# haotiansun14/rl-rep

Hardware: NVIDIA B200
Metric: agent updates/sec (higher is better)
Workload: dtype tf32

## Files before the change

### rlrep_b200/csrc/gemm_chain.cu

```cuda
#include <algorithm>
#include <cmath>
#include <cstdlib>
#include <cstring>

#include "common.cuh"
#include "gemm_chain.cuh"
#include "ptx.cuh"

namespace rlrep {

namespace {

constexpr int kThreads = 320;
constexpr int kEpiWarps = 8;
constexpr int kStages = 6;
constexpr int kCW = 16;
constexpr int kTwPitch = kCW + 4;
constexpr int kMaxBn = 128;
constexpr int kBM = 128, kBK = 32;
constexpr int kABytes = kBM * kBK * 4;
constexpr int kStageBytes = kABytes + kMaxBn * kBK * 4;
constexpr int kTbufFloats = kEpiWarps * 32 * kTwPitch;
constexpr int kSub = 4, kCtrStride = 32;
constexpr int kDbgItems = 16, kDbgEvents = 10;
constexpr int kSmemBytes = kStages * kStageBytes + 1024 + 256 + kTbufFloats * 4;
static_assert(kSmemBytes <= 227 * 1024, "chain kernel shared memory");

__device__ __forceinline__ void red_release_add(unsigned* p, unsigned v) {
  asm volatile("red.release.gpu.global.add.u32 [%0], %1;" ::"l"(p), "r"(v) : "memory");
}
__device__ __forceinline__ unsigned atom_add_acq_rel(unsigned* p, unsigned v) {
  unsigned old;
  asm volatile("atom.acq_rel.gpu.global.add.u32 %0, [%1], %2;" : "=r"(old) : "l"(p), "r"(v) : "memory");
  return old;
}
__device__ __forceinline__ void fence_proxy_async_global() { asm volatile("fence.proxy.async.global;" ::: "memory"); }
__device__ __forceinline__ void fence_tensormap_acquire(const CUtensorMap* m) {
  asm volatile("fence.proxy.tensormap::generic.acquire.gpu [%0], 128;" ::"l"(reinterpret_cast<uint64_t>(m)) : "memory");
}
__device__ __forceinline__ unsigned ld_relaxed(const unsigned* p) {
  unsigned v;
  asm volatile("ld.relaxed.gpu.global.u32 %0, [%1];" : "=r"(v) : "l"(p) : "memory");
  return v;
}
__device__ __forceinline__ void wait_counter(const unsigned* done, int dep, int dep_tiles) {
  const unsigned* p = done + (size_t)dep * kSub * kCtrStride;
  unsigned target[kSub];
#pragma unroll
  for (int sub = 0; sub < kSub; ++sub) target[sub] = (unsigned)((dep_tiles - sub + kSub - 1) / kSub);
  long long t0 = 0;
  while (true) {
    unsigned v[kSub];
#pragma unroll
    for (int sub = 0; sub < kSub; ++sub) v[sub] = ld_relaxed(p + sub * kCtrStride);
    bool ok = true;
#pragma unroll
    for (int sub = 0; sub < kSub; ++sub) ok = ok && v[sub] >= target[sub];
    if (ok) return;
    __nanosleep(20);
    if (t0 == 0) t0 = clock64();
    if (clock64() - t0 > 4000000000LL) {
      printf("rlrep: chain dependency wait timed out (block %d, gemm %d, tiles %d, counters %u %u %u %u)\n", blockIdx.x, dep,
             dep_tiles, v[0], v[1], v[2], v[3]);
      __trap();
    }
  }
}
__device__ __forceinline__ void fence_acquire_gpu() { asm volatile("fence.acq_rel.gpu;" ::: "memory"); }

__device__ __forceinline__ void epilogue_bar() { asm volatile("bar.sync 1, 256;" ::: "memory"); }

__device__ __forceinline__ float elu_fast(float x) {
  const float n = fminf(x, 0.f);
  float p = 1.f / 5040.f;
  p = fmaf(p, n, 1.f / 720.f);
  p = fmaf(p, n, 1.f / 120.f);
  p = fmaf(p, n, 1.f / 24.f);
  p = fmaf(p, n, 1.f / 6.f);
  p = fmaf(p, n, 0.5f);
  p = fmaf(p, n, 1.f);
  p *= n;
  const float e = __expf(n) - 1.f;
  const float r = n < -0.34657359f ? e : p;
  return x > 0.f ? x : r;
}

__device__ __forceinline__ bool aligned16(const void* p) { return (reinterpret_cast<uintptr_t>(p) & 15) == 0; }

__device__ __forceinline__ float chain_epilogue_scalar(const Epilogue& e, float acc, int m, int n, const float* cptr) {
  float v = acc * e.scale;
  if (e.r1_u) v = fmaf(__ldcg(e.r1_u + m), __ldcg(e.r1_v + n), v);
  if (e.bias) v += __ldg(e.bias + n);
  if (e.pre_out) e.pre_out[(size_t)m * e.ld_pre + n] = v;
  v = apply_act(v, e.act);
  if (e.dact != DACT_NONE) v *= apply_dact(__ldcg(e.aux + (size_t)m * e.ld_aux + n), e.dact);
  if (e.accumulate) v += __ldcg(cptr);
  return v;
}

struct ChunkOperands {
  float4 bias, r1v;
  float4 aux[4];
  float r1u[4];
};
__device__ __forceinline__ void chunk_prefetch(ChunkOperands& o, const Epilogue& epi, int M, int m_base, int gn0, int lane) {
  const int piece = lane & 3, rsub = lane >> 2;
  const int on = gn0 + 4 * piece;
  o.bias = make_float4(0.f, 0.f, 0.f, 0.f);
  o.r1v = make_float4(0.f, 0.f, 0.f, 0.f);
  if (epi.bias) o.bias = __ldg(reinterpret_cast<const float4*>(epi.bias + on));
  if (epi.r1_u) o.r1v = __ldcg(reinterpret_cast<const float4*>(epi.r1_v + on));
#pragma unroll
  for (int r4 = 0; r4 < 4; ++r4) {
    const int om = m_base + r4 * 8 + rsub;
    o.aux[r4] = make_float4(0.f, 0.f, 0.f, 0.f);
    o.r1u[r4] = 0.f;
    if (om < M) {
      if (epi.dact != DACT_NONE) o.aux[r4] = __ldcg(reinterpret_cast<const float4*>(epi.aux + (size_t)om * epi.ld_aux + on));
      if (epi.r1_u) o.r1u[r4] = __ldcg(epi.r1_u + om);
    }
  }
}

template <int ACT, int DACT>
__device__ __forceinline__ void chain_store_rows(const Epilogue& epi, const ChunkOperands& o, const float* tw,
                                                 float* __restrict__ C, int ldc, int M, int m_base, int gn0, int lane) {
  const int piece = lane & 3, rsub = lane >> 2;
  const int on = gn0 + 4 * piece;
#pragma unroll
  for (int r4 = 0; r4 < 4; ++r4) {
    const int r = r4 * 8 + rsub;
    const int om = m_base + r;
    if (om < M) {
      const float4 a4 = *reinterpret_cast<const float4*>(tw + r * kTwPitch + 4 * piece);
      float v[4] = {a4.x * epi.scale, a4.y * epi.scale, a4.z * epi.scale, a4.w * epi.scale};
      if (epi.r1_u) {
        const float u = o.r1u[r4];
        v[0] = fmaf(u, o.r1v.x, v[0]); v[1] = fmaf(u, o.r1v.y, v[1]); v[2] = fmaf(u, o.r1v.z, v[2]); v[3] = fmaf(u, o.r1v.w, v[3]);
      }
      v[0] += o.bias.x; v[1] += o.bias.y; v[2] += o.bias.z; v[3] += o.bias.w;
      if (epi.pre_out)
        *reinterpret_cast<float4*>(epi.pre_out + (size_t)om * epi.ld_pre + on) = make_float4(v[0], v[1], v[2], v[3]);
      if constexpr (ACT != ACT_NONE) {
#pragma unroll
        for (int e = 0; e < 4; ++e) v[e] = ACT == ACT_ELU ? elu_fast(v[e]) : apply_act(v[e], ACT < 0 ? epi.act : ACT);
      }
      if constexpr (DACT != DACT_NONE) {
        const int dact = DACT < 0 ? epi.dact : DACT;
        if (dact != DACT_NONE) {
          const float4 x = o.aux[r4];
          v[0] *= apply_dact(x.x, dact); v[1] *= apply_dact(x.y, dact); v[2] *= apply_dact(x.z, dact); v[3] *= apply_dact(x.w, dact);
        }
      }
      float4* cp = reinterpret_cast<float4*>(C + (size_t)om * ldc + on);
      if (epi.accumulate) {
        const float4 c0 = __ldcg(cp);
        v[0] += c0.x; v[1] += c0.y; v[2] += c0.z; v[3] += c0.w;
      }
      *cp = make_float4(v[0], v[1], v[2], v[3]);
    }
  }
}

__global__ void __launch_bounds__(kThreads, 1)
gemm_chain_kernel(const ChainGemmDesc* __restrict__ gemms, const ChainTask* __restrict__ tasks,
                  const int* __restrict__ task_begin, unsigned* __restrict__ done, unsigned* __restrict__ exit_ctr,
                  int n_gemms, unsigned long long* __restrict__ dbg) {
  auto stamp = [&](int item, int ev) {
    if (dbg != nullptr && item < kDbgItems) {
      unsigned long long t;
      asm volatile("mov.u64 %0, %%globaltimer;" : "=l"(t)::"memory");
      dbg[((size_t)blockIdx.x * kDbgItems + item) * kDbgEvents + ev] = t;
    }
  };
  if (threadIdx.x == 0) stamp(kDbgItems - 1, 2);
  extern __shared__ uint8_t smem_raw[];
  uint8_t* smem = reinterpret_cast<uint8_t*>((reinterpret_cast<uintptr_t>(smem_raw) + 1023) & ~uintptr_t(1023));
  uint64_t* full_bar = reinterpret_cast<uint64_t*>(smem + kStages * kStageBytes);
  uint64_t* empty_bar = full_bar + 8;
  uint64_t* acc_full = empty_bar + 8;
  uint64_t* acc_empty = acc_full + 2;
  uint32_t* tmem_slot = reinterpret_cast<uint32_t*>(acc_empty + 2);
  volatile unsigned* arrival = reinterpret_cast<volatile unsigned*>(tmem_slot + 1);
  float* tbuf = reinterpret_cast<float*>(smem + kStages * kStageBytes + 256);

  const int warp = threadIdx.x >> 5, lane = threadIdx.x & 31;
  const int t_begin = task_begin[blockIdx.x], t_end = task_begin[blockIdx.x + 1];

  if (threadIdx.x == 0) {
    for (int s = 0; s < kStages; ++s) {
      ptx::mbar_init(&full_bar[s], 1);
      ptx::mbar_init(&empty_bar[s], 1);
    }
    for (int a = 0; a < 2; ++a) {
      ptx::mbar_init(&acc_full[a], 1);
      ptx::mbar_init(&acc_empty[a], kEpiWarps);
    }
    ptx::fence_mbar_init();
  }
  if (warp == 1) {
    ptx::tmem_alloc(tmem_slot, 2 * kMaxBn);
    ptx::tmem_relinquish();
  }
  ptx::tc_fence_before_sync();
  __syncthreads();
  ptx::tc_fence_after_sync();
  const uint32_t tmem_base = *tmem_slot;
  ptx::pdl_wait();

  if (warp == 0) {
    if (lane == 0) {
      int it = 0, last_gemm = -1;
      for (int t = t_begin; t < t_end; ++t) {
        const ChainTask tk = tasks[t];
        const ChainGemmDesc* g = gemms + tk.gemm;
        const int n_deps = g->n_deps;
        const int bn = g->bn, a_mn = g->a_mn, b_mn = g->b_mn;
        const int m0 = (tk.tile % g->tiles_m) * kBM, n0 = (tk.tile / g->tiles_m) * bn;
        const int kb0 = tk.split * g->kb_per_split, kb1 = min(g->nkb, kb0 + g->kb_per_split);
        int dep_id[kChainMaxDeps], dep_tiles[kChainMaxDeps];
#pragma unroll
        for (int d = 0; d < kChainMaxDeps; ++d) {
          dep_id[d] = d < n_deps ? g->dep[d] : 0;
          dep_tiles[d] = d < n_deps ? (int)g->dep_target[d] : 0;
        }
        if (tk.gemm != last_gemm) {
          fence_tensormap_acquire(&g->tmA);
          fence_tensormap_acquire(&g->tmB);
          last_gemm = tk.gemm;
        }
        stamp(t - t_begin, 0);
        if (dbg != nullptr && t - t_begin < kDbgItems)
          dbg[((size_t)blockIdx.x * kDbgItems + (t - t_begin)) * kDbgEvents + 8] =
              (unsigned long long)tk.gemm | ((unsigned long long)tk.tile << 16) | ((unsigned long long)tk.split << 40);
#pragma unroll
        for (int d = 0; d < kChainMaxDeps; ++d)
          if (d < n_deps) wait_counter(done, dep_id[d], dep_tiles[d]);
        if (n_deps > 0) {
          fence_acquire_gpu();
          fence_proxy_async_global();
        }
        stamp(t - t_begin, 1);
        const uint32_t tx = kABytes + bn * kBK * 4;
        for (int kb = kb0; kb < kb1; ++kb, ++it) {
          const int s = it % kStages;
          ptx::mbar_wait(&empty_bar[s], ((it / kStages) & 1) ^ 1);
          ptx::mbar_arrive_expect_tx(&full_bar[s], tx);
          uint8_t* a_dst = smem + s * kStageBytes;
          uint8_t* b_dst = a_dst + kABytes;
          const int k0 = kb * kBK;
          if (!a_mn) ptx::tma_load_2d(a_dst, &g->tmA, &full_bar[s], k0, m0);
          else ptx::tma_load_3d(a_dst, &g->tmA, &full_bar[s], 0, k0, m0 / 32);
          if (!b_mn) ptx::tma_load_2d(b_dst, &g->tmB, &full_bar[s], k0, n0);
          else ptx::tma_load_3d(b_dst, &g->tmB, &full_bar[s], 0, k0, n0 / 32);
        }
        stamp(t - t_begin, 2);
      }
    }
  } else if (warp == 1) {
    if (ptx::elect_one()) {
      int it = 0, tc = 0;
      for (int t = t_begin; t < t_end; ++t, ++tc) {
        const ChainTask tk = tasks[t];
        const ChainGemmDesc* g = gemms + tk.gemm;
        const int bn = g->bn, a_mn = g->a_mn, b_mn = g->b_mn;
        const int kb0 = tk.split * g->kb_per_split, kb1 = min(g->nkb, kb0 + g->kb_per_split);
        const uint32_t idesc = ptx::make_idesc_tf32(kBM, bn, a_mn != 0, b_mn != 0);
        const int acc = tc & 1;
        ptx::mbar_wait(&acc_empty[acc], ((tc >> 1) & 1) ^ 1);
        ptx::tc_fence_after_sync();
        const uint32_t d_tmem = tmem_base + acc * kMaxBn;
        for (int kb = kb0; kb < kb1; ++kb, ++it) {
          const int s = it % kStages;
          ptx::mbar_wait(&full_bar[s], (it / kStages) & 1);
          if (kb == kb0) stamp(t - t_begin, 3);
          ptx::tc_fence_after_sync();
          const uint32_t a_addr = ptx::smem_u32(smem + s * kStageBytes);
          const uint32_t b_addr = a_addr + kABytes;
#pragma unroll
          for (int k = 0; k < kBK / 8; ++k) {
            const uint64_t adesc = a_mn ? ptx::make_smem_desc(a_addr + k * 1024, 4096, 512, 1)
                                        : ptx::make_smem_desc(a_addr + k * 32, 16, 1024, 2);
            const uint64_t bdesc = b_mn ? ptx::make_smem_desc(b_addr + k * 1024, 4096, 512, 1)
                                        : ptx::make_smem_desc(b_addr + k * 32, 16, 1024, 2);
            ptx::mma_tf32_ss(d_tmem, adesc, bdesc, idesc, (kb > kb0 || k > 0) ? 1u : 0u);
          }
          ptx::mma_commit(&empty_bar[s]);
        }
        ptx::mma_commit(&acc_full[acc]);
        stamp(t - t_begin, 4);
      }
    }
  } else {
    const int q = warp & 3, half = (warp - 2) >> 2;
    float* tw = tbuf + (warp - 2) * (32 * kTwPitch);
    int tc = 0;
    for (int t = t_begin; t < t_end; ++t, ++tc) {
      const ChainTask tk = tasks[t];
      const ChainGemmDesc* g = gemms + tk.gemm;
      const Epilogue epi = g->epi;
      const int bn = g->bn, M = g->M, N = g->N, ldc = g->ldc, split_k = g->split_k;
      float* __restrict__ C = g->C;
      float* __restrict__ ws = g->ws;
      unsigned* __restrict__ tile_ctr = g->tile_ctr;
      const int m0 = (tk.tile % g->tiles_m) * kBM, n0 = (tk.tile / g->tiles_m) * bn;
      const int chunks = bn / kCW;
      const int acc = tc & 1;
      const uint32_t t_acc = tmem_base + (static_cast<uint32_t>(32 * q) << 16) + acc * kMaxBn;
      const int row = 32 * q + lane;
      ptx::mbar_wait(&acc_full[acc], (tc >> 1) & 1);
      if (threadIdx.x == 64) stamp(t - t_begin, 5);
      ptx::tc_fence_after_sync();

      bool final = true;
      const size_t part_floats = (size_t)kBM * bn;
      float* ws_tile = split_k > 1 ? ws + (size_t)tk.tile * split_k * part_floats : nullptr;
      const bool dist = split_k > 1 && g->dist != 0;
      int c_first = half, c_step = 2;
      if (split_k > 1) {
        float* part = ws_tile + (size_t)tk.split * part_floats;
#pragma unroll 1
        for (int c = half; c < chunks; c += 2) {
          if (dist && c % split_k == tk.split) continue;
          uint32_t v[kCW];
          ptx::tmem_ld_32x32b_x16(t_acc + c * kCW, v);
          ptx::tmem_ld_wait();
#pragma unroll
          for (int j = 0; j < kCW / 4; ++j)
            __stcg(reinterpret_cast<float4*>(part + ((size_t)(c * (kCW / 4) + j) * kBM + row) * 4),
                   make_float4(__uint_as_float(v[4 * j]), __uint_as_float(v[4 * j + 1]), __uint_as_float(v[4 * j + 2]),
                               __uint_as_float(v[4 * j + 3])));
        }
        epilogue_bar();
        if (threadIdx.x == 64) {
          unsigned* ctr = tile_ctr + tk.tile;
          const unsigned old = atom_add_acq_rel(ctr, 1u);
          if (dist) {
            if (old + 1 < (unsigned)split_k) {
              unsigned long long t0 = 0;
              unsigned spins = 0;
              while (ld_relaxed(ctr) < (unsigned)split_k) {
                __nanosleep(20);
                if ((++spins & 0xfff) == 0) {
                  unsigned long long now;
                  asm volatile("mov.u64 %0, %%globaltimer;" : "=l"(now));
                  if (t0 == 0) t0 = now;
                  else if (now - t0 > 2000000000ull) __trap();
                }
              }
              fence_acquire_gpu();
            }
          } else if (old == (unsigned)(split_k - 1)) {
            *ctr = 0;
          }
          *arrival = old;
          stamp(t - t_begin, 6);
        }
        epilogue_bar();
        final = dist || *arrival == (unsigned)(split_k - 1);
        if (dist) {
          c_first = tk.split + split_k * half;
          c_step = 2 * split_k;
        }
      }
      if (final) {
        const bool use_aux = epi.dact != DACT_NONE;
        const bool vec_ok = (ldc & 3) == 0 && aligned16(C) && (N & 3) == 0 &&
                            (!use_aux || ((epi.ld_aux & 3) == 0 && aligned16(epi.aux))) &&
                            (!epi.pre_out || ((epi.ld_pre & 3) == 0 && aligned16(epi.pre_out))) &&
                            (!epi.bias || aligned16(epi.bias)) && (!epi.r1_v || aligned16(epi.r1_v));
#pragma unroll 1
        for (int c = c_first; c < chunks; c += c_step) {
          const int gn0 = n0 + c * kCW;
          const bool fast = vec_ok && gn0 + kCW <= N;
          ChunkOperands ops;
          if (fast) chunk_prefetch(ops, epi, M, m0 + 32 * q, gn0, lane);
          float a[kCW];
          if (split_k == 1) {
            uint32_t v[kCW];
            ptx::tmem_ld_32x32b_x16(t_acc + c * kCW, v);
            ptx::tmem_ld_wait();
#pragma unroll
            for (int e = 0; e < kCW; ++e) a[e] = __uint_as_float(v[e]);
          } else {
            const float* base = ws_tile + ((size_t)(c * (kCW / 4)) * kBM + row) * 4;
            float4 nxt[kCW / 4];
            const int s_first = tk.split == 0 ? 1 : 0;
#pragma unroll
            for (int j = 0; j < kCW / 4; ++j)
              nxt[j] = __ldcg(reinterpret_cast<const float4*>(base + (size_t)s_first * part_floats + (size_t)j * kBM * 4));
#pragma unroll 1
            for (int s = 0; s < split_k; ++s) {
              if (s == tk.split) {
                uint32_t v[kCW];
                ptx::tmem_ld_32x32b_x16(t_acc + c * kCW, v);
                ptx::tmem_ld_wait();
                if (s == 0) {
#pragma unroll
                  for (int e = 0; e < kCW; ++e) a[e] = __uint_as_float(v[e]);
                } else {
#pragma unroll
                  for (int e = 0; e < kCW; ++e) a[e] += __uint_as_float(v[e]);
                }
                continue;
              }
              float4 cur[kCW / 4];
#pragma unroll
              for (int j = 0; j < kCW / 4; ++j) cur[j] = nxt[j];
              int s2 = s + 1;
              if (s2 == tk.split) ++s2;
              if (s2 < split_k) {
#pragma unroll
                for (int j = 0; j < kCW / 4; ++j)
                  nxt[j] = __ldcg(reinterpret_cast<const float4*>(base + (size_t)s2 * part_floats + (size_t)j * kBM * 4));
              }
              if (s == 0) {
#pragma unroll
                for (int j = 0; j < kCW / 4; ++j) { a[4 * j] = cur[j].x; a[4 * j + 1] = cur[j].y; a[4 * j + 2] = cur[j].z; a[4 * j + 3] = cur[j].w; }
              } else {
#pragma unroll
                for (int j = 0; j < kCW / 4; ++j) { a[4 * j] += cur[j].x; a[4 * j + 1] += cur[j].y; a[4 * j + 2] += cur[j].z; a[4 * j + 3] += cur[j].w; }
              }
            }
          }
#pragma unroll
          for (int j = 0; j < kCW / 4; ++j)
            *reinterpret_cast<float4*>(tw + lane * kTwPitch + 4 * j) = make_float4(a[4 * j], a[4 * j + 1], a[4 * j + 2], a[4 * j + 3]);
          __syncwarp();
          if (fast) {
#define RLREP_CSTORE(A, D) chain_store_rows<A, D>(epi, ops, tw, C, ldc, M, m0 + 32 * q, gn0, lane)
            RLREP_EPILOGUE_SWITCH(epi, RLREP_CSTORE);
#undef RLREP_CSTORE
          } else if (gn0 < N) {
            const int piece = lane & 3, rsub = lane >> 2;
#pragma unroll 1
            for (int r4 = 0; r4 < 4; ++r4) {
              const int r = r4 * 8 + rsub, om = m0 + 32 * q + r;
              if (om >= M) continue;
#pragma unroll 1
              for (int e = 0; e < 4; ++e) {
                const int on = gn0 + 4 * piece + e;
                if (on < N) {
                  float* cp = C + (size_t)om * ldc + on;
                  *cp = chain_epilogue_scalar(epi, tw[r * kTwPitch + 4 * piece + e], om, on, cp);
                }
              }
            }
          }
          __syncwarp();
        }
        if (threadIdx.x == 64) stamp(t - t_begin, 9);
        epilogue_bar();
        if (threadIdx.x == 64) {
          fence_proxy_async_global();
          const int pub = dist ? tk.tile * split_k + tk.split : tk.tile;
          red_release_add(done + ((size_t)tk.gemm * kSub + (pub % kSub)) * kCtrStride, 1u);
          stamp(t - t_begin, 7);
          if (dist) {
            unsigned* ctr = tile_ctr + tk.tile;
            if (atomicAdd(ctr, 1u) == (unsigned)(2 * split_k - 1)) *ctr = 0;
          }
        }
      }
      ptx::tc_fence_before_sync();
      __syncwarp();
      if (lane == 0) ptx::mbar_arrive(&acc_empty[acc]);
    }
  }
  ptx::pdl_launch_dependents();
  ptx::tc_fence_before_sync();
  __syncthreads();
  if (warp == 1) ptx::tmem_dealloc(tmem_base, 2 * kMaxBn);
  if (threadIdx.x == 0) {
    const unsigned old = atom_add_acq_rel(exit_ctr, 1u);
    if (old == gridDim.x - 1) {
      for (int i = 0; i < n_gemms * kSub; ++i) done[(size_t)i * kCtrStride] = 0;
      *exit_ctr = 0;
      __threadfence();
    }
    stamp(kDbgItems - 1, 3);
  }
}

struct Range {
  uintptr_t lo = 0, hi = 0;
  bool overlaps(const Range& o) const { return lo < o.hi && o.lo < hi && lo != hi && o.lo != o.hi; }
};
Range range_of(const float* p, long long rows, long long ld, long long cols) {
  Range r;
  if (p == nullptr || rows <= 0 || cols <= 0) return r;
  r.lo = reinterpret_cast<uintptr_t>(p);
  r.hi = r.lo + (size_t)((rows - 1) * ld + cols) * sizeof(float);
  return r;
}
struct Footprint {
  std::vector<Range> reads, writes;
};
Footprint footprint(const GemmArgs& a) {
  Footprint f;
  f.reads.push_back(a.a_mn ? range_of(a.A, a.K, a.lda, a.M) : range_of(a.A, a.M, a.lda, a.K));
  f.reads.push_back(a.b_mn ? range_of(a.B, a.K, a.ldb, a.N) : range_of(a.B, a.N, a.ldb, a.K));
  f.reads.push_back(range_of(a.epi.bias, 1, 0, a.N));
  f.reads.push_back(range_of(a.epi.r1_u, 1, 0, a.M));
  f.reads.push_back(range_of(a.epi.r1_v, 1, 0, a.N));
  if (a.epi.dact != DACT_NONE) f.reads.push_back(range_of(a.epi.aux, a.M, a.epi.ld_aux, a.N));
  f.writes.push_back(range_of(a.C, a.M, a.ldc, a.N));
  if (a.epi.accumulate) f.reads.push_back(f.writes.back());
  f.writes.push_back(range_of(a.epi.pre_out, a.M, a.epi.ld_pre, a.N));
  return f;
}
bool conflicts(const Footprint& earlier, const Footprint& later) {
  for (const Range& w : earlier.writes) {
    for (const Range& r : later.reads)
      if (w.overlaps(r)) return true;
    for (const Range& r : later.writes)
      if (w.overlaps(r)) return true;
  }
  for (const Range& w : later.writes)
    for (const Range& r : earlier.reads)
      if (w.overlaps(r)) return true;
  return false;
}

unsigned long long* g_chain_dbg = nullptr;

int env_int(const char* name, int dflt) {
  const char* e = std::getenv(name);
  return e ? std::atoi(e) : dflt;
}

bool dist_possible(int bn, int split) { return split > 1 && (bn / kCW) % split == 0; }
double plan_cost(int tiles, int nkb, int bn, int split, int share, bool dist) {
  const int kb_per = ceil_div(nkb, split);
  const double kb_bytes = kABytes + bn * kBK * 4;
  const double waves = std::ceil((double)tiles * split / share);
  const double stream = waves * kb_per * kb_bytes / 150e3;
  const double chip = (double)tiles * split * kb_per * kb_bytes / 12e6;
  if (dist) {
    return 1.5 + std::max(stream, chip) + waves * (0.25 * ceil_div(bn, 64) + 1.0 + 1.0 * ceil_div(bn / split, 64)) +
           0.1 * (split - 1);
  }
  double t = 1.5 + std::max(stream, chip) + waves * 1.0 * ceil_div(bn, 64);
  if (split > 1) t += 1.5 + 0.3 * (split - 1) * ceil_div(bn, 64);
  return t;
}

}

void set_chain_debug_buffer(unsigned long long* dev) { g_chain_dbg = dev; }

bool chain_eligible(const GemmArgs& a) {
  return tc_eligible(a) && a.conv_w == 0 && a.M >= 32 && a.N >= 32 && a.K >= 8;
}

GemmChain::~GemmChain() {
  if (dev_) cudaFree(dev_);
}

bool GemmChain::matches(const std::vector<GemmArgs>& seq) const {
  if (seq.size() != seq_.size()) return false;
  for (size_t i = 0; i < seq.size(); ++i) {
    const GemmArgs &x = seq[i], &y = seq_[i];
    if (x.M != y.M || x.N != y.N || x.K != y.K || x.A != y.A || x.B != y.B || x.C != y.C || x.lda != y.lda ||
        x.ldb != y.ldb || x.ldc != y.ldc || x.a_mn != y.a_mn || x.b_mn != y.b_mn || x.epi.bias != y.epi.bias ||
        x.epi.r1_u != y.epi.r1_u || x.epi.r1_v != y.epi.r1_v || x.epi.aux != y.epi.aux || x.epi.pre_out != y.epi.pre_out ||
        x.epi.ld_aux != y.epi.ld_aux || x.epi.ld_pre != y.epi.ld_pre || x.epi.act != y.epi.act || x.epi.dact != y.epi.dact ||
        x.epi.accumulate != y.epi.accumulate || x.epi.scale != y.epi.scale)
      return false;
  }
  return true;
}

void GemmChain::build(const std::vector<GemmArgs>& seq, int force_bn, int force_split) {
  RLREP_CHECK(dev_ == nullptr, "chain already built");
  RLREP_CHECK(!seq.empty(), "empty chain");
  const int n = (int)seq.size();
  for (const GemmArgs& a : seq) RLREP_CHECK(chain_eligible(a), "GEMM cannot be a member of a chain");
  seq_ = seq;
  int n_sm = kNumSMs;
  {
    int dev = 0;
    RLREP_CUDA(cudaGetDevice(&dev));
    RLREP_CUDA(cudaDeviceGetAttribute(&n_sm, cudaDevAttrMultiProcessorCount, dev));
  }
  static bool attr_set = false;
  if (!attr_set) {
    RLREP_CUDA(cudaFuncSetAttribute(gemm_chain_kernel, cudaFuncAttributeMaxDynamicSharedMemorySize, kSmemBytes));
    attr_set = true;
  }
  int per_sm = 0;
  RLREP_CUDA(cudaOccupancyMaxActiveBlocksPerMultiprocessor(&per_sm, gemm_chain_kernel, kThreads, kSmemBytes));
  RLREP_CHECK(per_sm >= 1, "chain kernel does not fit on an SM");
  const int n_cta = n_sm;

  std::vector<Footprint> fp(n);
  for (int i = 0; i < n; ++i) fp[i] = footprint(seq[i]);
  std::vector<std::vector<int>> deps(n);
  std::vector<std::vector<char>> reach(n, std::vector<char>(n, 0));
  std::vector<int> level(n, 0);
  for (int j = 0; j < n; ++j) {
    std::vector<int> direct;
    for (int i = 0; i < j; ++i)
      if (conflicts(fp[i], fp[j])) direct.push_back(i);
    for (int i : direct) {
      reach[j][i] = 1;
      for (int k = 0; k < n; ++k)
        if (reach[i][k]) reach[j][k] = 1;
    }
    for (int i : direct) {
      bool implied = false;
      for (int k : direct)
        if (k != i && reach[k][i]) implied = true;
      if (!implied) deps[j].push_back(i);
      level[j] = std::max(level[j], level[i] + 1);
    }
    RLREP_CHECK((int)deps[j].size() <= kChainMaxDeps, "a chain GEMM has too many direct dependencies");
  }
  levels_ = 1 + *std::max_element(level.begin(), level.end());

  std::vector<int> bn(n), split(n), share(n), first_cta(n), dist(n, 0);
  const int dist_mode = env_int("RLREP_CHAIN_DIST", 1);
  auto work_of = [&](int i) {
    return (double)ceil_div(seq[i].M, kBM) * ceil_div(seq[i].N, kMaxBn) * ceil_div(seq[i].K, kBK);
  };
  auto items_of = [&](int i) { return ceil_div(seq[i].M, kBM) * ceil_div(seq[i].N, bn[i]) * (dist[i] ? split[i] : 1); };
  for (int L = 0; L < levels_; ++L) {
    std::vector<int> members;
    for (int i = 0; i < n; ++i)
      if (level[i] == L) members.push_back(i);
    double total = 0.0;
    for (int i : members) total += work_of(i);
    int cursor = 0, seen = 0;
    for (int i : members) {
      const GemmArgs& a = seq[i];
      const int nkb = ceil_div(a.K, kBK);
      ++seen;
      int sh = std::max(4, (int)std::floor(n_cta * work_of(i) / total));
      if (seen == (int)members.size()) sh = std::max(sh, n_cta - cursor);
      sh = std::min(sh, n_cta);
      first_cta[i] = cursor % n_cta;
      cursor += sh;
      share[i] = sh;
      double best = 1e300;
      for (int cbn : {32, 64, 128}) {
        if (force_bn && cbn != force_bn) continue;
        if (!force_bn && cbn > 32 && cbn / 2 >= a.N) continue;
        const int tiles = ceil_div(a.M, kBM) * ceil_div(a.N, cbn);
        for (int s : {1, 2, 4, 8, 16}) {
          if (force_split && s != force_split) continue;
          if (s > 1 && (s - 1) * ceil_div(nkb, s) >= nkb) continue;
          for (int d = 0; d < 2; ++d) {
            if (d == 1 && (dist_mode == 0 || !dist_possible(cbn, s) || tiles * s > sh)) continue;
            if (d == 0 && dist_mode == 2 && dist_possible(cbn, s) && tiles * s <= sh) continue;
            const double c = plan_cost(tiles, nkb, cbn, s, sh, d == 1);
            if (c < best - 1e-9) {
              best = c;
              bn[i] = cbn;
              split[i] = s;
              dist[i] = d;
            }
          }
        }
      }
      if (best > 1e299) {
        bn[i] = force_bn ? force_bn : 32;
        split[i] = 1;
        dist[i] = 0;
      }
    }
  }

  std::vector<std::vector<ChainTask>> per_cta(n_cta);
  std::vector<int> order(n);
  for (int i = 0; i < n; ++i) order[i] = i;
  std::stable_sort(order.begin(), order.end(), [&](int x, int y) { return level[x] < level[y]; });
  size_t ws_floats = 0, ctr_count = 0;
  std::vector<size_t> ws_off(n, 0), ctr_off(n, 0);
  std::vector<ChainGemmDesc> descs(n);
  bytes_ = flops_ = 0.0;
  for (int i : order) {
    const GemmArgs& a = seq[i];
    const int tiles_m = ceil_div(a.M, kBM), tiles_n = ceil_div(a.N, bn[i]);
    const int tiles = tiles_m * tiles_n;
    int item = 0;
    for (int t = 0; t < tiles; ++t)
      for (int s = 0; s < split[i]; ++s, ++item)
        per_cta[(first_cta[i] + item % share[i]) % n_cta].push_back(ChainTask{i, t, s, 0});
    ChainGemmDesc& d = descs[i];
    std::memset(&d, 0, sizeof(d));
    d.tmA = make_operand_map(a.A, a.a_mn, a.M, a.K, a.lda, kBM);
    d.tmB = make_operand_map(a.B, a.b_mn, a.N, a.K, a.ldb, bn[i]);
    d.epi = a.epi;
    d.C = a.C;
    d.ldc = a.ldc; d.M = a.M; d.N = a.N; d.K = a.K;
    d.bn = bn[i]; d.a_mn = a.a_mn; d.b_mn = a.b_mn; d.nkb = ceil_div(a.K, kBK);
    d.split_k = split[i]; d.kb_per_split = ceil_div(d.nkb, split[i]);
    d.dist = dist[i];
    d.tiles_m = tiles_m; d.tiles_n = tiles_n;
    d.n_deps = (int)deps[i].size();
    for (int k = 0; k < d.n_deps; ++k) {
      const int j = deps[i][k];
      d.dep[k] = j;
      d.dep_target[k] = (unsigned)items_of(j);
    }
    ctr_off[i] = ctr_count;
    ctr_count += (size_t)tiles;
    if (split[i] > 1) {
      ws_off[i] = ws_floats;
      ws_floats += (size_t)tiles * split[i] * kBM * bn[i];
    }
    bytes_ += 4.0 * ((double)a.M * a.K + (double)a.N * a.K + (double)a.M * a.N);
    flops_ += 2.0 * a.M * a.N * a.K;
  }
  std::vector<ChainTask> tasks;
  std::vector<int> begin(n_cta + 1, 0);
  for (int c = 0; c < n_cta; ++c) {
    begin[c] = (int)tasks.size();
    tasks.insert(tasks.end(), per_cta[c].begin(), per_cta[c].end());
  }
  begin[n_cta] = (int)tasks.size();
  grid_ = n_cta;

  auto up = [](size_t x) { return (x + 255) & ~size_t(255); };
  const size_t o_desc = 0;
  const size_t o_tasks = up(o_desc + sizeof(ChainGemmDesc) * n);
  const size_t o_begin = up(o_tasks + sizeof(ChainTask) * tasks.size());
  const size_t o_done = up(o_begin + sizeof(int) * begin.size());
  const size_t o_exit = up(o_done + sizeof(unsigned) * n * kSub * kCtrStride);
  const size_t o_ctr = up(o_exit + sizeof(unsigned));
  const size_t o_ws = up(o_ctr + sizeof(unsigned) * ctr_count);
  const size_t total_bytes = o_ws + sizeof(float) * ws_floats + 256;
  RLREP_CUDA(cudaMalloc(&dev_, total_bytes));
  RLREP_CUDA(cudaMemset(dev_, 0, o_ws));
  char* base = static_cast<char*>(dev_);
  d_gemms_ = reinterpret_cast<ChainGemmDesc*>(base + o_desc);
  d_tasks_ = reinterpret_cast<ChainTask*>(base + o_tasks);
  d_task_begin_ = reinterpret_cast<int*>(base + o_begin);
  d_done_ = reinterpret_cast<unsigned*>(base + o_done);
  d_exit_ = reinterpret_cast<unsigned*>(base + o_exit);
  for (int i = 0; i < n; ++i) {
    descs[i].tile_ctr = reinterpret_cast<unsigned*>(base + o_ctr) + ctr_off[i];
    descs[i].ws = split[i] > 1 ? reinterpret_cast<float*>(base + o_ws) + ws_off[i] : nullptr;
  }
  RLREP_CUDA(cudaMemcpy(d_gemms_, descs.data(), sizeof(ChainGemmDesc) * n, cudaMemcpyHostToDevice));
  RLREP_CUDA(cudaMemcpy(d_tasks_, tasks.data(), sizeof(ChainTask) * tasks.size(), cudaMemcpyHostToDevice));
  RLREP_CUDA(cudaMemcpy(d_task_begin_, begin.data(), sizeof(int) * begin.size(), cudaMemcpyHostToDevice));
  RLREP_CUDA(cudaDeviceSynchronize());
  if (env_int("RLREP_CHAIN_VERBOSE", 0)) {
    std::fprintf(stderr, "rlrep chain: %d GEMMs, %d levels, %zu items, ws %.1f MB\n", n, levels_, tasks.size(),
                 ws_floats * 4 / 1e6);
    for (int i = 0; i < n; ++i)
      std::fprintf(stderr, "  [%d] L%d M=%d N=%d K=%d a_mn=%d b_mn=%d bn=%d split=%d%s share=%d deps=%d\n", i, level[i],
                   seq[i].M, seq[i].N, seq[i].K, (int)seq[i].a_mn, (int)seq[i].b_mn, bn[i], split[i],
                   dist[i] ? " (distributed)" : "", share[i], (int)deps[i].size());
  }
}

void GemmChain::launch(cudaStream_t stream) {
  RLREP_CHECK(dev_ != nullptr, "chain not built");
  cudaLaunchConfig_t cfg = {};
  cfg.gridDim = dim3(grid_);
  cfg.blockDim = dim3(kThreads);
  cfg.dynamicSmemBytes = kSmemBytes;
  cfg.stream = stream;
  cudaLaunchAttribute attr[2];
  attr[0].id = cudaLaunchAttributeCooperative;
  attr[0].val.cooperative = 1;
  attr[1] = pdl_attribute();
  cfg.attrs = attr;
  cfg.numAttrs = 2;
  RLREP_CUDA(cudaLaunchKernelEx(&cfg, gemm_chain_kernel, (const ChainGemmDesc*)d_gemms_, (const ChainTask*)d_tasks_,
                                (const int*)d_task_begin_, d_done_, d_exit_, (int)seq_.size(), g_chain_dbg));
  RLREP_LAUNCHED_W("gemm_chain", stream, bytes_, flops_);
}

}
```

### rlrep_b200/csrc/gemm_chain.cuh

```cuda
#pragma once
#include <vector>

#include "gemm.cuh"

namespace rlrep {

constexpr int kChainMaxDeps = 6;

struct alignas(128) ChainGemmDesc {
  CUtensorMap tmA;
  CUtensorMap tmB;
  Epilogue epi;
  int dist;
  float* C;
  float* ws;
  unsigned* tile_ctr;
  int ldc, M, N, K;
  int bn, a_mn, b_mn, nkb;
  int split_k, kb_per_split, tiles_m, tiles_n;
  int n_deps;
  int dep[kChainMaxDeps];
  unsigned dep_target[kChainMaxDeps];
};

struct ChainTask {
  int gemm, tile, split, pad;
};

class GemmChain {
 public:
  GemmChain() = default;
  GemmChain(const GemmChain&) = delete;
  GemmChain& operator=(const GemmChain&) = delete;
  ~GemmChain();
  bool matches(const std::vector<GemmArgs>& seq) const;
  void build(const std::vector<GemmArgs>& seq, int force_bn = 0, int force_split = 0);
  void launch(cudaStream_t stream);
  int size() const { return (int)seq_.size(); }
  int levels() const { return levels_; }

 private:
  std::vector<GemmArgs> seq_;
  void* dev_ = nullptr;
  ChainGemmDesc* d_gemms_ = nullptr;
  ChainTask* d_tasks_ = nullptr;
  int* d_task_begin_ = nullptr;
  unsigned* d_done_ = nullptr;
  unsigned* d_exit_ = nullptr;
  int grid_ = 0, levels_ = 0;
  double bytes_ = 0.0, flops_ = 0.0;
};

void set_chain_debug_buffer(unsigned long long* dev);

bool chain_eligible(const GemmArgs& a);

}
```

Baseline: 1321.

## Replace whole-GEMM dependency counters with per-tile-band counters in chain kernel

Each GEMM's completion is now tracked per (M-tile, 128-column band) counter instead of four striped whole-GEMM counters. The host computes, for every work item, exactly which producer bands its A/B/epilogue operands read, so a consumer tile can start once only the rows and columns it needs are finished. Producers it cannot map this way still wait on all of that producer's bands. The warp-0 producer now polls dependencies cooperatively across lanes with __all_sync, and the last CTA resets the counters in parallel. This is meant to cut pipeline bubbles between chained GEMM levels, at the cost of more counters, per-item dependency lists and extra host-side analysis.

```diff
diff --git a/rlrep_b200/csrc/gemm_chain.cu b/rlrep_b200/csrc/gemm_chain.cu
--- a/rlrep_b200/csrc/gemm_chain.cu
+++ b/rlrep_b200/csrc/gemm_chain.cu
@@ -21,7 +21,7 @@
 constexpr int kABytes = kBM * kBK * 4;
 constexpr int kStageBytes = kABytes + kMaxBn * kBK * 4;
 constexpr int kTbufFloats = kEpiWarps * 32 * kTwPitch;
-constexpr int kSub = 4, kCtrStride = 32;
+constexpr int kCtrStride = 32;
 constexpr int kDbgItems = 16, kDbgEvents = 10;
 constexpr int kSmemBytes = kStages * kStageBytes + 1024 + 256 + kTbufFloats * 4;
 static_assert(kSmemBytes <= 227 * 1024, "chain kernel shared memory");
@@ -43,30 +43,29 @@
   asm volatile("ld.relaxed.gpu.global.u32 %0, [%1];" : "=r"(v) : "l"(p) : "memory");
   return v;
 }
-__device__ __forceinline__ void wait_counter(const unsigned* done, int dep, int dep_tiles) {
-  const unsigned* p = done + (size_t)dep * kSub * kCtrStride;
-  unsigned target[kSub];
-#pragma unroll
-  for (int sub = 0; sub < kSub; ++sub) target[sub] = (unsigned)((dep_tiles - sub + kSub - 1) / kSub);
-  long long t0 = 0;
-  while (true) {
-    unsigned v[kSub];
-#pragma unroll
-    for (int sub = 0; sub < kSub; ++sub) v[sub] = ld_relaxed(p + sub * kCtrStride);
-    bool ok = true;
-#pragma unroll
-    for (int sub = 0; sub < kSub; ++sub) ok = ok && v[sub] >= target[sub];
-    if (ok) return;
-    __nanosleep(20);
-    if (t0 == 0) t0 = clock64();
-    if (clock64() - t0 > 4000000000LL) {
-      printf("rlrep: chain dependency wait timed out (block %d, gemm %d, tiles %d, counters %u %u %u %u)\n", blockIdx.x, dep,
-             dep_tiles, v[0], v[1], v[2], v[3]);
-      __trap();
-    }
-  }
-}
 __device__ __forceinline__ void fence_acquire_gpu() { asm volatile("fence.acq_rel.gpu;" ::: "memory"); }
+
+__device__ __forceinline__ void wait_deps(const unsigned* done, const ChainDep* deps, int n_deps, int lane) {
+  for (int base = 0; base < n_deps; base += 32) {
+    const bool mine = base + lane < n_deps;
+    const ChainDep d = mine ? deps[base + lane] : ChainDep{0u, 0u};
+    const unsigned* p = done + (size_t)d.ctr * kCtrStride;
+    long long t0 = 0;
+    while (true) {
+      const unsigned v = mine ? ld_relaxed(p) : 0u;
+      if (__all_sync(0xffffffffu, v >= d.target)) break;
+      __nanosleep(20);
+      if (t0 == 0) t0 = clock64();
+      if (clock64() - t0 > 4000000000LL) {
+        if (v < d.target)
+          printf("rlrep: chain dependency wait timed out (block %d, counter %u at %u of %u)\n", blockIdx.x, d.ctr, v,
+                 d.target);
+        __trap();
+      }
+    }
+  }
+  if (n_deps > 0) fence_acquire_gpu();
+}
 
 __device__ __forceinline__ void epilogue_bar() { asm volatile("bar.sync 1, 256;" ::: "memory"); }
 
@@ -164,8 +163,8 @@
 
 __global__ void __launch_bounds__(kThreads, 1)
 gemm_chain_kernel(const ChainGemmDesc* __restrict__ gemms, const ChainTask* __restrict__ tasks,
-                  const int* __restrict__ task_begin, unsigned* __restrict__ done, unsigned* __restrict__ exit_ctr,
-                  int n_gemms, unsigned long long* __restrict__ dbg) {
+                  const ChainDep* __restrict__ deps, const int* __restrict__ task_begin, unsigned* __restrict__ done,
+                  unsigned* __restrict__ exit_ctr, int n_ctrs, unsigned long long* __restrict__ dbg) {
   auto stamp = [&](int item, int ev) {
     if (dbg != nullptr && item < kDbgItems) {
       unsigned long long t;
@@ -209,37 +208,28 @@
   ptx::pdl_wait();
 
   if (warp == 0) {
-    if (lane == 0) {
-      int it = 0, last_gemm = -1;
-      for (int t = t_begin; t < t_end; ++t) {
-        const ChainTask tk = tasks[t];
-        const ChainGemmDesc* g = gemms + tk.gemm;
-        const int n_deps = g->n_deps;
-        const int bn = g->bn, a_mn = g->a_mn, b_mn = g->b_mn;
-        const int m0 = (tk.tile % g->tiles_m) * kBM, n0 = (tk.tile / g->tiles_m) * bn;
-        const int kb0 = tk.split * g->kb_per_split, kb1 = min(g->nkb, kb0 + g->kb_per_split);
-        int dep_id[kChainMaxDeps], dep_tiles[kChainMaxDeps];
-#pragma unroll
-        for (int d = 0; d < kChainMaxDeps; ++d) {
-          dep_id[d] = d < n_deps ? g->dep[d] : 0;
-          dep_tiles[d] = d < n_deps ? (int)g->dep_target[d] : 0;
-        }
+    int it = 0, last_gemm = -1;
+    for (int t = t_begin; t < t_end; ++t) {
+      const ChainTask tk = tasks[t];
+      const ChainGemmDesc* g = gemms + tk.gemm;
+      const int bn = g->bn, a_mn = g->a_mn, b_mn = g->b_mn;
+      const int m0 = (tk.tile % g->tiles_m) * kBM, n0 = (tk.tile / g->tiles_m) * bn;
+      const int kb0 = tk.split * g->kb_per_split, kb1 = min(g->nkb, kb0 + g->kb_per_split);
+      if (lane == 0) {
         if (tk.gemm != last_gemm) {
           fence_tensormap_acquire(&g->tmA);
           fence_tensormap_acquire(&g->tmB);
-          last_gemm = tk.gemm;
         }
         stamp(t - t_begin, 0);
         if (dbg != nullptr && t - t_begin < kDbgItems)
           dbg[((size_t)blockIdx.x * kDbgItems + (t - t_begin)) * kDbgEvents + 8] =
               (unsigned long long)tk.gemm | ((unsigned long long)tk.tile << 16) | ((unsigned long long)tk.split << 40);
-#pragma unroll
-        for (int d = 0; d < kChainMaxDeps; ++d)
-          if (d < n_deps) wait_counter(done, dep_id[d], dep_tiles[d]);
-        if (n_deps > 0) {
-          fence_acquire_gpu();
-          fence_proxy_async_global();
-        }
+      }
+      last_gemm = tk.gemm;
+      wait_deps(done, deps + tk.dep_begin, tk.n_deps, lane);
+      __syncwarp();
+      if (lane == 0) {
+        if (tk.n_deps > 0) fence_proxy_async_global();
         stamp(t - t_begin, 1);
         const uint32_t tx = kABytes + bn * kBK * 4;
         for (int kb = kb0; kb < kb1; ++kb, ++it) {
@@ -256,6 +246,7 @@
         }
         stamp(t - t_begin, 2);
       }
+      __syncwarp();
     }
   } else if (warp == 1) {
     if (ptx::elect_one()) {
@@ -304,6 +295,7 @@
       float* __restrict__ ws = g->ws;
       unsigned* __restrict__ tile_ctr = g->tile_ctr;
       const int m0 = (tk.tile % g->tiles_m) * kBM, n0 = (tk.tile / g->tiles_m) * bn;
+      const int band_ctr = g->band_ctr + (tk.tile % g->tiles_m) * g->n_bands + n0 / kChainBand;
       const int chunks = bn / kCW;
       const int acc = tc & 1;
       const uint32_t t_acc = tmem_base + (static_cast<uint32_t>(32 * q) << 16) + acc * kMaxBn;
@@ -453,8 +445,7 @@
         epilogue_bar();
         if (threadIdx.x == 64) {
           fence_proxy_async_global();
-          const int pub = dist ? tk.tile * split_k + tk.split : tk.tile;
-          red_release_add(done + ((size_t)tk.gemm * kSub + (pub % kSub)) * kCtrStride, 1u);
+          red_release_add(done + (size_t)band_ctr * kCtrStride, 1u);
           stamp(t - t_begin, 7);
           if (dist) {
             unsigned* ctr = tile_ctr + tk.tile;
@@ -471,15 +462,14 @@
   ptx::tc_fence_before_sync();
   __syncthreads();
   if (warp == 1) ptx::tmem_dealloc(tmem_base, 2 * kMaxBn);
-  if (threadIdx.x == 0) {
-    const unsigned old = atom_add_acq_rel(exit_ctr, 1u);
-    if (old == gridDim.x - 1) {
-      for (int i = 0; i < n_gemms * kSub; ++i) done[(size_t)i * kCtrStride] = 0;
-      *exit_ctr = 0;
-      __threadfence();
-    }
-    stamp(kDbgItems - 1, 3);
-  }
+  if (threadIdx.x == 0) *arrival = atom_add_acq_rel(exit_ctr, 1u);
+  __syncthreads();
+  if (*arrival == gridDim.x - 1) {
+    for (int i = threadIdx.x; i < n_ctrs; i += kThreads) done[(size_t)i * kCtrStride] = 0;
+    if (threadIdx.x == 0) *exit_ctr = 0;
+    __threadfence();
+  }
+  if (threadIdx.x == 0) stamp(kDbgItems - 1, 3);
 }
 
 struct Range {
@@ -522,6 +512,52 @@
   return false;
 }
 
+struct Rect {
+  const float* p;
+  long long ld, r0, r1, c0, c1;
+};
+std::vector<Rect> item_rects(const GemmArgs& a, long long m0, long long m1, long long n0, long long n1, long long k0,
+                             long long k1) {
+  std::vector<Rect> r;
+  r.push_back(a.a_mn ? Rect{a.A, a.lda, k0, k1, m0, m1} : Rect{a.A, a.lda, m0, m1, k0, k1});
+  r.push_back(a.b_mn ? Rect{a.B, a.ldb, k0, k1, n0, n1} : Rect{a.B, a.ldb, n0, n1, k0, k1});
+  if (a.epi.bias) r.push_back(Rect{a.epi.bias, 0, 0, 1, n0, n1});
+  if (a.epi.r1_u) r.push_back(Rect{a.epi.r1_u, 0, 0, 1, m0, m1});
+  if (a.epi.r1_v) r.push_back(Rect{a.epi.r1_v, 0, 0, 1, n0, n1});
+  if (a.epi.dact != DACT_NONE) r.push_back(Rect{a.epi.aux, a.epi.ld_aux, m0, m1, n0, n1});
+  r.push_back(Rect{a.C, a.ldc, m0, m1, n0, n1});
+  if (a.epi.pre_out) r.push_back(Rect{a.epi.pre_out, a.epi.ld_pre, m0, m1, n0, n1});
+  return r;
+}
+bool map_onto(const Rect& r, const GemmArgs& p, long long& r0, long long& r1, long long& c0, long long& c1) {
+  r0 = r1 = c0 = c1 = 0;
+  if (r.r1 <= r.r0 || r.c1 <= r.c0) return true;
+  const long long rows = r.r1 - r.r0;
+  if (!range_of(r.p + r.r0 * r.ld + r.c0, rows, r.ld, r.c1 - r.c0).overlaps(range_of(p.C, p.M, p.ldc, p.N))) return true;
+  const long long off = r.p - p.C;
+  if (off < 0 || (rows > 1 && r.ld != p.ldc) || off % p.ldc + r.c1 > p.ldc) return false;
+  r0 = std::max(0LL, off / p.ldc + r.r0);
+  r1 = std::min((long long)p.M, off / p.ldc + r.r1);
+  c0 = std::max(0LL, off % p.ldc + r.c0);
+  c1 = std::min((long long)p.N, off % p.ldc + r.c1);
+  if (r1 <= r0 || c1 <= c0) r0 = r1 = c0 = c1 = 0;
+  return true;
+}
+bool band_waits(const GemmArgs& p, const Footprint& fp_p, const GemmArgs& c, const Footprint& fp_c) {
+  const Range pre = range_of(p.epi.pre_out, p.M, p.epi.ld_pre, p.N);
+  for (const Range& x : fp_c.reads)
+    if (x.overlaps(pre)) return false;
+  for (const Range& w : fp_c.writes) {
+    if (w.overlaps(pre)) return false;
+    for (const Range& x : fp_p.reads)
+      if (w.overlaps(x)) return false;
+  }
+  long long r0, r1, c0, c1;
+  for (const Rect& r : item_rects(c, 0, c.M, 0, c.N, 0, c.K))
+    if (!map_onto(r, p, r0, r1, c0, c1)) return false;
+  return true;
+}
+
 unsigned long long* g_chain_dbg = nullptr;
 
 int env_int(const char* name, int dflt) {
@@ -595,11 +631,11 @@
 
   std::vector<Footprint> fp(n);
   for (int i = 0; i < n; ++i) fp[i] = footprint(seq[i]);
-  std::vector<std::vector<int>> deps(n);
+  std::vector<std::vector<int>> deps(n), direct_of(n);
   std::vector<std::vector<char>> reach(n, std::vector<char>(n, 0));
   std::vector<int> level(n, 0);
   for (int j = 0; j < n; ++j) {
-    std::vector<int> direct;
+    std::vector<int>& direct = direct_of[j];
     for (int i = 0; i < j; ++i)
       if (conflicts(fp[i], fp[j])) direct.push_back(i);
     for (int i : direct) {
@@ -614,7 +650,6 @@
       if (!implied) deps[j].push_back(i);
       level[j] = std::max(level[j], level[i] + 1);
     }
-    RLREP_CHECK((int)deps[j].size() <= kChainMaxDeps, "a chain GEMM has too many direct dependencies");
   }
   levels_ = 1 + *std::max_element(level.begin(), level.end());
 
@@ -623,7 +658,6 @@
   auto work_of = [&](int i) {
     return (double)ceil_div(seq[i].M, kBM) * ceil_div(seq[i].N, kMaxBn) * ceil_div(seq[i].K, kBK);
   };
-  auto items_of = [&](int i) { return ceil_div(seq[i].M, kBM) * ceil_div(seq[i].N, bn[i]) * (dist[i] ? split[i] : 1); };
   for (int L = 0; L < levels_; ++L) {
     std::vector<int> members;
     for (int i = 0; i < n; ++i)
@@ -676,6 +710,48 @@
   std::stable_sort(order.begin(), order.end(), [&](int x, int y) { return level[x] < level[y]; });
   size_t ws_floats = 0, ctr_count = 0;
   std::vector<size_t> ws_off(n, 0), ctr_off(n, 0);
+  std::vector<int> band_ctr(n), n_bands(n);
+  std::vector<unsigned> band_target;
+  for (int i = 0; i < n; ++i) {
+    const int tiles_n = ceil_div(seq[i].N, bn[i]), per_band = kChainBand / bn[i];
+    band_ctr[i] = (int)band_target.size();
+    n_bands[i] = ceil_div(seq[i].N, kChainBand);
+    for (int tm = 0; tm < ceil_div(seq[i].M, kBM); ++tm)
+      for (int b = 0; b < n_bands[i]; ++b)
+        band_target.push_back((unsigned)(std::min(per_band, tiles_n - b * per_band) * (dist[i] ? split[i] : 1)));
+  }
+  n_ctrs_ = (int)band_target.size();
+  std::vector<std::vector<char>> banded(n, std::vector<char>(n, 0));
+  for (int j = 0; j < n; ++j)
+    for (int i : direct_of[j]) banded[j][i] = band_waits(seq[i], fp[i], seq[j], fp[j]);
+  auto item_deps = [&](const ChainTask& tk, std::vector<ChainDep>& out) {
+    const int j = tk.gemm;
+    const GemmArgs& a = seq[j];
+    const int tiles_m = ceil_div(a.M, kBM), nkb = ceil_div(a.K, kBK), kb_per = ceil_div(nkb, split[j]);
+    const long long m0 = (long long)(tk.tile % tiles_m) * kBM, n0 = (long long)(tk.tile / tiles_m) * bn[j];
+    const long long k0 = (long long)tk.split * kb_per * kBK;
+    const std::vector<Rect> rects = item_rects(a, m0, std::min<long long>(m0 + kBM, a.M), n0,
+                                               std::min<long long>(n0 + bn[j], a.N), k0,
+                                               std::min<long long>(k0 + (long long)kb_per * kBK, a.K));
+    std::vector<int> ctrs;
+    for (int i : direct_of[j]) {
+      const int first = band_ctr[i], nb = n_bands[i];
+      if (!banded[j][i]) {
+        for (int c = 0; c < ceil_div(seq[i].M, kBM) * nb; ++c) ctrs.push_back(first + c);
+        continue;
+      }
+      for (const Rect& r : rects) {
+        long long r0, r1, c0, c1;
+        map_onto(r, seq[i], r0, r1, c0, c1);
+        if (r1 <= r0) continue;
+        for (long long tm = r0 / kBM; tm <= (r1 - 1) / kBM; ++tm)
+          for (long long b = c0 / kChainBand; b <= (c1 - 1) / kChainBand; ++b) ctrs.push_back(first + (int)(tm * nb + b));
+      }
+    }
+    std::sort(ctrs.begin(), ctrs.end());
+    ctrs.erase(std::unique(ctrs.begin(), ctrs.end()), ctrs.end());
+    for (int c : ctrs) out.push_back(ChainDep{(unsigned)c, band_target[c]});
+  };
   std::vector<ChainGemmDesc> descs(n);
   bytes_ = flops_ = 0.0;
   for (int i : order) {
@@ -685,7 +761,7 @@
     int item = 0;
     for (int t = 0; t < tiles; ++t)
       for (int s = 0; s < split[i]; ++s, ++item)
-        per_cta[(first_cta[i] + item % share[i]) % n_cta].push_back(ChainTask{i, t, s, 0});
+        per_cta[(first_cta[i] + item % share[i]) % n_cta].push_back(ChainTask{i, t, s, 0, 0});
     ChainGemmDesc& d = descs[i];
     std::memset(&d, 0, sizeof(d));
     d.tmA = make_operand_map(a.A, a.a_mn, a.M, a.K, a.lda, kBM);
@@ -697,12 +773,7 @@
     d.split_k = split[i]; d.kb_per_split = ceil_div(d.nkb, split[i]);
     d.dist = dist[i];
     d.tiles_m = tiles_m; d.tiles_n = tiles_n;
-    d.n_deps = (int)deps[i].size();
-    for (int k = 0; k < d.n_deps; ++k) {
-      const int j = deps[i][k];
-      d.dep[k] = j;
-      d.dep_target[k] = (unsigned)items_of(j);
-    }
+    d.band_ctr = band_ctr[i]; d.n_bands = n_bands[i];
     ctr_off[i] = ctr_count;
     ctr_count += (size_t)tiles;
     if (split[i] > 1) {
@@ -713,10 +784,18 @@
     flops_ += 2.0 * a.M * a.N * a.K;
   }
   std::vector<ChainTask> tasks;
-  std::vector<int> begin(n_cta + 1, 0);
+  std::vector<ChainDep> dep_list;
+  std::vector<int> begin(n_cta + 1, 0), waits_min(n, 1 << 30), waits_max(n, 0);
   for (int c = 0; c < n_cta; ++c) {
     begin[c] = (int)tasks.size();
-    tasks.insert(tasks.end(), per_cta[c].begin(), per_cta[c].end());
+    for (ChainTask tk : per_cta[c]) {
+      tk.dep_begin = (int)dep_list.size();
+      item_deps(tk, dep_list);
+      tk.n_deps = (int)dep_list.size() - tk.dep_begin;
+      waits_min[tk.gemm] = std::min(waits_min[tk.gemm], tk.n_deps);
+      waits_max[tk.gemm] = std::max(waits_max[tk.gemm], tk.n_deps);
+      tasks.push_back(tk);
+    }
   }
   begin[n_cta] = (int)tasks.size();
   grid_ = n_cta;
@@ -724,9 +803,10 @@
   auto up = [](size_t x) { return (x + 255) & ~size_t(255); };
   const size_t o_desc = 0;
   const size_t o_tasks = up(o_desc + sizeof(ChainGemmDesc) * n);
-  const size_t o_begin = up(o_tasks + sizeof(ChainTask) * tasks.size());
+  const size_t o_deps = up(o_tasks + sizeof(ChainTask) * tasks.size());
+  const size_t o_begin = up(o_deps + sizeof(ChainDep) * dep_list.size());
   const size_t o_done = up(o_begin + sizeof(int) * begin.size());
-  const size_t o_exit = up(o_done + sizeof(unsigned) * n * kSub * kCtrStride);
+  const size_t o_exit = up(o_done + sizeof(unsigned) * n_ctrs_ * kCtrStride);
   const size_t o_ctr = up(o_exit + sizeof(unsigned));
   const size_t o_ws = up(o_ctr + sizeof(unsigned) * ctr_count);
   const size_t total_bytes = o_ws + sizeof(float) * ws_floats + 256;
@@ -735,6 +815,7 @@
   char* base = static_cast<char*>(dev_);
   d_gemms_ = reinterpret_cast<ChainGemmDesc*>(base + o_desc);
   d_tasks_ = reinterpret_cast<ChainTask*>(base + o_tasks);
+  d_deps_ = reinterpret_cast<ChainDep*>(base + o_deps);
   d_task_begin_ = reinterpret_cast<int*>(base + o_begin);
   d_done_ = reinterpret_cast<unsigned*>(base + o_done);
   d_exit_ = reinterpret_cast<unsigned*>(base + o_exit);
@@ -744,15 +825,22 @@
   }
   RLREP_CUDA(cudaMemcpy(d_gemms_, descs.data(), sizeof(ChainGemmDesc) * n, cudaMemcpyHostToDevice));
   RLREP_CUDA(cudaMemcpy(d_tasks_, tasks.data(), sizeof(ChainTask) * tasks.size(), cudaMemcpyHostToDevice));
+  if (!dep_list.empty())
+    RLREP_CUDA(cudaMemcpy(d_deps_, dep_list.data(), sizeof(ChainDep) * dep_list.size(), cudaMemcpyHostToDevice));
   RLREP_CUDA(cudaMemcpy(d_task_begin_, begin.data(), sizeof(int) * begin.size(), cudaMemcpyHostToDevice));
   RLREP_CUDA(cudaDeviceSynchronize());
   if (env_int("RLREP_CHAIN_VERBOSE", 0)) {
-    std::fprintf(stderr, "rlrep chain: %d GEMMs, %d levels, %zu items, ws %.1f MB\n", n, levels_, tasks.size(),
-                 ws_floats * 4 / 1e6);
-    for (int i = 0; i < n; ++i)
-      std::fprintf(stderr, "  [%d] L%d M=%d N=%d K=%d a_mn=%d b_mn=%d bn=%d split=%d%s share=%d deps=%d\n", i, level[i],
-                   seq[i].M, seq[i].N, seq[i].K, (int)seq[i].a_mn, (int)seq[i].b_mn, bn[i], split[i],
-                   dist[i] ? " (distributed)" : "", share[i], (int)deps[i].size());
+    std::fprintf(stderr, "rlrep chain: %d GEMMs, %d levels, %zu items, %d band counters, ws %.1f MB\n", n, levels_,
+                 tasks.size(), n_ctrs_, ws_floats * 4 / 1e6);
+    for (int i = 0; i < n; ++i) {
+      int whole = 0;
+      for (int k : direct_of[i]) whole += !banded[i][k];
+      std::fprintf(stderr,
+                   "  [%d] L%d M=%d N=%d K=%d a_mn=%d b_mn=%d bn=%d split=%d%s share=%d deps=%d (%d whole) waits on "
+                   "%d..%d counters\n",
+                   i, level[i], seq[i].M, seq[i].N, seq[i].K, (int)seq[i].a_mn, (int)seq[i].b_mn, bn[i], split[i],
+                   dist[i] ? " (distributed)" : "", share[i], (int)direct_of[i].size(), whole, waits_min[i], waits_max[i]);
+    }
   }
 }
 
@@ -770,7 +858,8 @@
   cfg.attrs = attr;
   cfg.numAttrs = 2;
   RLREP_CUDA(cudaLaunchKernelEx(&cfg, gemm_chain_kernel, (const ChainGemmDesc*)d_gemms_, (const ChainTask*)d_tasks_,
-                                (const int*)d_task_begin_, d_done_, d_exit_, (int)seq_.size(), g_chain_dbg));
+                                (const ChainDep*)d_deps_, (const int*)d_task_begin_, d_done_, d_exit_, n_ctrs_,
+                                g_chain_dbg));
   RLREP_LAUNCHED_W("gemm_chain", stream, bytes_, flops_);
 }
 
diff --git a/rlrep_b200/csrc/gemm_chain.cuh b/rlrep_b200/csrc/gemm_chain.cuh
--- a/rlrep_b200/csrc/gemm_chain.cuh
+++ b/rlrep_b200/csrc/gemm_chain.cuh
@@ -5,7 +5,7 @@
 
 namespace rlrep {
 
-constexpr int kChainMaxDeps = 6;
+constexpr int kChainBand = 128;
 
 struct alignas(128) ChainGemmDesc {
   CUtensorMap tmA;
@@ -18,13 +18,16 @@
   int ldc, M, N, K;
   int bn, a_mn, b_mn, nkb;
   int split_k, kb_per_split, tiles_m, tiles_n;
-  int n_deps;
-  int dep[kChainMaxDeps];
-  unsigned dep_target[kChainMaxDeps];
+  int band_ctr, n_bands;
+};
+
+struct ChainDep {
+  unsigned ctr, target;
 };
 
 struct ChainTask {
-  int gemm, tile, split, pad;
+  int gemm, tile, split;
+  int dep_begin, n_deps;
 };
 
 class GemmChain {
@@ -44,10 +47,11 @@
   void* dev_ = nullptr;
   ChainGemmDesc* d_gemms_ = nullptr;
   ChainTask* d_tasks_ = nullptr;
+  ChainDep* d_deps_ = nullptr;
   int* d_task_begin_ = nullptr;
   unsigned* d_done_ = nullptr;
   unsigned* d_exit_ = nullptr;
-  int grid_ = 0, levels_ = 0;
+  int grid_ = 0, levels_ = 0, n_ctrs_ = 0;
   double bytes_ = 0.0, flops_ = 0.0;
 };
 
```

Result: slower. 1264 (median of 6 runs) (-4.2%).
